# kendallsullivan/mcmc_spec

Hardware: AMD Instinct MI355X
Metric: walker log-likelihood evals/sec (whole node) (higher is better)
Workload: dtype f64

## Files before the change

mcmc_spec_amd/csrc/msx.hip:

```cpp

#include <dlfcn.h>
#include <hip/hip_runtime.h>
#include <math.h>
#include <stdint.h>
#include <stdio.h>
#include <string.h>

#include <algorithm>
#include <array>
#include <mutex>
#include <type_traits>
#include <string>
#include <vector>

#include "../../include/msx.h"

#include "dev_types.h"
#include "wave_ops.h"
#include "blend.h"
#include "recipe.h"
#include "median.h"
#include "logprob_kernel.h"
#include "move_kernels.h"
#include "tempered_kernels.h"
// ... 34 lines not shown
    bool pf_ok = false;
    bool pf256_ok = false;
    bool model_in_global = false;
    void *rccl_comm = nullptr;
    hipStream_t comm_stream = nullptr;
    hipEvent_t ev_ready = nullptr;
    hipEvent_t ev_done[4] = {nullptr, nullptr, nullptr, nullptr};
    int comm_world = 0, comm_rank = 0;
    std::vector<msx_ctx *> loop_peers;
    hipEvent_t loop_eval_done = nullptr;
    hipEvent_t loop_copied = nullptr;
    double *d_model_scratch = nullptr;
    SegPart *d_segparts = nullptr;
    unsigned long long *d_seg_flag = nullptr;
    int nseg = 1;
    int64_t scratch_rows = 0;
    int32_t path = 0;
    int32_t broaden_placement = 0;
    double *d_raw_win = nullptr;
    int64_t raw_i0 = 0, raw_n = 0;
    int raw_lx = 0;
    double raw_dx = 0.0, raw_sigma = 0.0;
    bool grid_rotated = false;
    int32_t ncomp = 1;
    InpathRec *d_inp_rec = nullptr;
    double *d_inp_tmp = nullptr, *d_inp_given = nullptr;
    const int64_t *d_pix_lo = nullptr;
    int64_t inp_rows = 0, inp_gstride = 0;
    int64_t pair_rows = 0;
    int64_t pair_min_walkers = 4096;
    int32_t *d_pair_plan = nullptr;
    PairItem *d_pair_items = nullptr;
    PairRec *d_pair_singles = nullptr;
    int32_t *h_pair_stats = nullptr;
    int64_t pair_auto_launches = 0;
    int32_t linked = -1;
    bool linked_poisoned = false;
    bool recipe_fast = false;
    unsigned char *d_recipe_block = nullptr;
    struct SamplerRun *smp = nullptr;
    struct OptRun *opt_run = nullptr;
    struct TemperedRun *tmp = nullptr;
    bool smp_overlap_launch = false;
    bool probe_launch = false;
    int32_t last_form = 0;
    int32_t smp_overlap_policy = -1;
    int32_t store_dtype = MSX_STORE_F64;
    bool store_f32 = false;
    uint64_t prob_gen = 0;
    std::vector<struct msx_group *> groups;
    bool products_staged = false;
    ProdMember PM;
    ProdMember *d_prod_member = nullptr;
    std::vector<void *> prod_allocs;
    char *d_prod_buf = nullptr;
    size_t prod_buf_bytes = 0;
};
static void sampler_free(msx_ctx *c);
static void opt_run_free(msx_ctx *c);
static void tempered_free(msx_ctx *c);

struct msx_group {
    int device = 0;
    std::string err;
    std::vector<msx_ctx *> members;
    std::vector<uint64_t> gen;
// ... 94 lines not shown
    if (count <= 0) {
        HIP_TRY(c, hipMalloc((void **)out, 16));
        if (track) track->push_back(*out);
        return MSX_OK;
    }
    HIP_TRY(c, hipMalloc((void **)out, sizeof(T) * count));
    if (track) track->push_back(*out);
    HIP_TRY(c, hipMemcpy(*out, host, sizeof(T) * count, hipMemcpyHostToDevice));
    return MSX_OK;
}

void free_problem(msx_ctx *c) {
    sampler_free(c);
    opt_run_free(c);
    tempered_free(c);
    for (msx_group *g : c->groups) group_run_drain(g);
    ++c->prob_gen;
    for (void *p : c->prob_allocs) (void)hipFree(p);
    c->prob_allocs.clear();
    c->problem_staged = false;
    for (void *p : c->prod_allocs) (void)hipFree(p);
    c->prod_allocs.clear();
    if (c->d_prod_buf) (void)hipFree(c->d_prod_buf);
    c->d_prod_buf = nullptr; c->prod_buf_bytes = 0;
    c->d_prod_member = nullptr;
    c->products_staged = false;
    if (c->d_opt_flux) (void)hipFree(c->d_opt_flux);
    if (c->d_opt_med) (void)hipFree(c->d_opt_med);
    c->d_opt_flux = c->d_opt_med = nullptr;
    c->opt_chains = 0;
    if (c->h_pair_stats) (void)hipHostFree(c->h_pair_stats);
    c->h_pair_stats = nullptr;
    void *sp[] = {c->d_model_scratch, c->d_segparts, c->d_seg_flag, c->d_pair_plan, c->d_pair_items, c->d_pair_singles,
                  c->d_inp_rec, c->d_inp_tmp, c->d_inp_given};
    for (void *p : sp)
        if (p) (void)hipFree(p);
    c->d_segparts = nullptr; c->d_seg_flag = nullptr; c->d_model_scratch = nullptr; c->scratch_rows = 0;
    c->d_pair_plan = nullptr; c->d_pair_items = nullptr; c->d_pair_singles = nullptr; c->pair_rows = 0;
    c->linked_poisoned = false;
    c->d_inp_rec = nullptr; c->d_inp_tmp = c->d_inp_given = nullptr; c->d_pix_lo = nullptr; c->inp_rows = 0;
}

void free_grid(msx_ctx *c) {
    void *ptrs[] = {c->d_grid, c->d_wl, c->d_kgrid, c->d_teff, c->d_logg, c->d_present};
    for (void *p : ptrs)
        if (p) (void)hipFree(p);
    c->d_grid = c->d_wl = c->d_kgrid = c->d_teff = c->d_logg = nullptr;
    c->d_present = nullptr;
    if (c->d_raw_win) (void)hipFree(c->d_raw_win);
    c->d_raw_win = nullptr; c->raw_n = 0;
    c->grid_rotated = false;
    c->ncomp = 1;
    c->grid_staged = false;
}

int64_t grid_rows(const msx_ctx *c) { return (int64_t)c->ncomp * c->nt * c->ng; }

int conv_taps(double mean_wl, double dx, double resolution, double maxsig, double *sigma_out, int *lx_out) {
    const double fwhm = 1.0 / resolution * mean_wl;
    const double sigma = fwhm / (2.0 * sqrt(2.0 * log(2.0)));
    const int lx = (int)(((sigma * maxsig) / dx) * 2.0) + 1;
    *sigma_out = sigma;
    *lx_out = lx;
    return lx;
}

int check_even_spacing(msx_ctx *c, const double *wl, int64_t n) {
    double mx = -INFINITY, mn = INFINITY, sum = 0.0;
    for (int64_t i = 1; i < n; ++i) {
        const double d = wl[i] - wl[i - 1];
        mx = d > mx ? d : mx;
// ... 152 lines not shown
    return {(const void *)logprob_kernel<NS, T, GM, SH, PF, LK, R32, FULL, GIVEN>, NS, T, GM, SH, PF, LK, R32, FULL, GIVEN, what};
}
const Variant kVariants[] = {
    variant<2, 256, false, false, false, false>("three workgroups per CU"),
    variant<2, 256, false, true, false, false>("two per CU, four pixels per lane and trip"),
    variant<2, 256, false, true, true, false>("two per CU, u / flux staged in LDS during the recipe, four pixels per lane and trip"),
    variant<2, 512, false, false, false, false>("one workgroup per CU, four pixels per lane and trip"),
    variant<2, 512, false, true, false, false>("<= 128 VGPRs: two workgroups fit a CU; rows one star at a time"),
    variant<2, 512, false, false, true, false>("one workgroup per CU, u / flux staged in LDS during the recipe, four pixels per lane and trip"),
    variant<3, 256, false, false, false, false>("three workgroups per CU"),
    variant<3, 512, false, false, false, false>("one workgroup per CU, four pixels per lane and trip"),
    variant<3, 512, false, false, true, false>("one workgroup per CU, u / flux staged in LDS during the recipe, four pixels per lane and trip"),
    variant<2, 512, false, false, false, true>("one workgroup per walker and 8192-pixel segment; partial sums and histogram counters exchanged inside the launch; the segment's data flux staged in LDS; four pixels per lane and trip"),
    variant<3, 512, false, false, false, true>("one workgroup per walker and 8192-pixel segment; partial sums and histogram counters exchanged inside the launch; the segment's data flux staged in LDS; four pixels per lane and trip"),
    variant<2, 512, true, false, false, false>("model vector in global memory (spectra beyond the LDS), sub-batched"),
    variant<3, 512, true, false, false, false>("model vector in global memory (spectra beyond the LDS), sub-batched"),
    variant<2, 256, false, false, false, false, true>("three workgroups per CU; R table stored in float32"),
    variant<2, 256, false, true, false, false, true>("two per CU, four pixels per lane and trip; R table stored in float32"),
    variant<2, 256, false, true, true, false, true>("two per CU, u / flux staged in LDS during the recipe, four pixels per lane and trip; R table stored in float32"),
    variant<2, 512, false, false, false, false, true>("one workgroup per CU, four pixels per lane and trip; R table stored in float32"),
    variant<2, 512, false, true, false, false, true>("<= 128 VGPRs: two workgroups fit a CU; rows one star at a time; R table stored in float32"),
    variant<2, 512, false, false, true, false, true>("one workgroup per CU, u / flux staged in LDS during the recipe, four pixels per lane and trip; R table stored in float32"),
    variant<2, 256, false, false, false, false, false, 3>("three workgroups per CU; whole trips, no clamps"),
    variant<2, 256, false, true, false, false, false, 3>("two per CU, four pixels per lane and trip; whole trips, no clamps"),
    variant<2, 256, false, true, true, false, false, 3>("two per CU, u / flux staged in LDS during the recipe, four pixels per lane and trip; whole trips, no clamps"),
    variant<2, 512, false, false, true, false, false, 2>("one workgroup per CU, u / flux staged in LDS during the recipe, four pixels per lane and trip; whole trips, no clamps in the chi^2 pass"),
    variant<2, 512, false, true, false, false, false, 2>("<= 128 VGPRs: two workgroups fit a CU; rows one star at a time; whole trips, no clamps in the chi^2 pass"),
    variant<2, 512, false, false, true, false, true, 2>("float32-stored grid table R; one workgroup per CU, u / flux staged in LDS; whole trips, no clamps in the chi^2 pass"),
    variant<2, 512, false, false, false, true, false, 2>("linked: one workgroup per walker and 8192-pixel segment; whole trips, no clamps in the chi^2 pass"),
    variant<2, 512, false, false, false, false, false, 0, true>("model values given by the in-path broadening kernels; four pixels per lane and trip"),
};

struct PairVariant {
    void (*fn)(const double *, const unsigned char *, int, int, int64_t, double, double, const int32_t *, DevProblem, double *, int32_t *);
    int nt;
    bool full;
};
const PairVariant kPairVariants[] = {
    {logprob_pair_kernel<512, 2, true>, 2, false},
    {logprob_pair_kernel<512, 2, true, true>, 2, true},
    {logprob_pair_kernel<512, 4, true>, 4, false},
    {logprob_pair_kernel<512, 4, true, true>, 4, true},
};

const Variant *find_variant(const Variant &want, bool whole) {
    const Variant *hit = nullptr;
    for (const Variant &v : kVariants)
        if (v.ns == want.ns && v.threads == want.threads && v.gm == want.gm && v.sh == want.sh && v.pf == want.pf &&
            v.lk == want.lk && v.r32 == want.r32 && v.given == want.given && (v.full == 0 || whole) && (!hit || v.full != 0))
            hit = &v;
    return hit;
}

struct LaunchPlan {
    int64_t rows = 0;
    int64_t m = 0;
    int block = 0;
    const Variant *v = nullptr;
    const PairVariant *pv = nullptr;
    const void *fn = nullptr;
    int threads = 0;
    size_t dyn_lds = 0;
    int64_t grid = 0;
    int64_t bytes = 0;
};


// ... 201 lines not shown
            pf = pf && g->pf_ok[m];
            pf256 = pf256 && g->pf256_ok[m];
        }
    const int B = block_threads > 0 ? block_threads : pick_block(g->cus, total, npix);
    bool whole = true;
    for (int m = 0; m < k; ++m)
        if (counts[m] > 0) whole = whole && whole_trips(g->probs[m], 2 * (int64_t)B);
    FusedShape want = fused_shape(g->cus, total, npix, B, shared512, pf, pf256);
    const int ns = g->nspec == 2 ? 2 : 3;
    const GroupVariant *hit = nullptr;
    for (int attempt = 0; attempt < 2 && !hit; ++attempt) {
        if (attempt == 1) want.sh = want.pf = false;
        for (const GroupVariant &v : kGroupVariants)
            if (v.ns == ns && v.threads == B && v.sh == want.sh && v.pf == want.pf && (v.full == 0 || whole) && (!hit || v.full != 0))
                hit = &v;
    }
    return hit ? group_plan_lds(g, counts, total, hit) : GroupPlan();
}

GroupPlan group_plan_lds(const msx_group *g, const int64_t *counts, int64_t total, const GroupVariant *v) {
    GroupPlan pl;
    pl.v = v;
    double bytes = 0.0;
    for (int m = 0; m < (int)g->members.size(); ++m) {
        if (counts[m] <= 0) continue;
        pl.dyn_lds = std::max(pl.dyn_lds, fused_dyn_lds(g->probs[m], v->pf));
        bytes += (double)fused_bytes(g->probs[m], v->pf, false) * (double)counts[m];
    }
    pl.bytes = (int64_t)(bytes / (double)total + 0.5);
    return pl;
}

int launch_pair(msx_ctx *c, const DevProblem &P, const LaunchArgs &A, const LaunchPlan &pl) {
    const int32_t *plan = c->d_pair_plan;
    hipLaunchKernelGGL(pair_plan_kernel, dim3((unsigned)((A.n + kPlanThreads - 1) / kPlanThreads)), dim3(kPlanThreads), 0, A.s, A.theta,
                       (const unsigned char *)c->d_recipe_block, A.niso_nt, A.ng_mode_fast, (int64_t)A.n, P.tmin, P.tmax,
                       c->d_pair_plan, c->d_pair_items, c->d_pair_singles, A.logp, A.status, c->h_pair_stats, P);
    HIP_TRY(c, hipGetLastError());
    hipLaunchKernelGGL(pl.pv->fn, dim3((unsigned)pl.grid), dim3((unsigned)pl.threads), 0, A.s, A.theta, (const unsigned char *)c->d_recipe_block,
                       A.niso_nt, A.ng_mode_fast, (int64_t)A.n, P.tmin, P.tmax, plan, P, A.logp, A.status);
    HIP_TRY(c, hipGetLastError());
    return MSX_OK;
}

hipError_t raise_one(const void *kernel) {
    hipFuncAttributes at;
    hipError_t e = hipFuncGetAttributes(&at, kernel);
    if (e != hipSuccess) return e;
    const int room = (160 * 1024 - (int)at.sharedSizeBytes) & ~15;
    return hipFuncSetAttribute(kernel, hipFuncAttributeMaxDynamicSharedMemorySize, room);
}
hipError_t raise_all() {
    hipError_t e = hipSuccess;
    for (const Variant &v : kVariants)
        if (e == hipSuccess && !v.gm) e = raise_one(v.fn);
    for (const GroupVariant &v : kGroupVariants) {
        if (e == hipSuccess) e = raise_one(v.fn);
        if (e == hipSuccess && v.smp_fn) e = raise_one(v.smp_fn);
    }
    if (e == hipSuccess) e = raise_one((const void *)broaden_conv_kernel);
    if (e == hipSuccess) e = raise_one((const void *)rot_broaden_kernel<true>);
    return e;
}
constexpr int kMaxDevices = 64;
int raise_dynamic_lds_limits(msx_ctx *c) {
    static std::mutex mu;
    static bool done[kMaxDevices] = {};
    if (c->device < 0 || c->device >= kMaxDevices)
        return fail(c, MSX_ERR_INVALID, "device index beyond the per-device table of dynamic-LDS limits (64 devices)");
    std::lock_guard<std::mutex> lock(mu);
    if (done[c->device]) return MSX_OK;
    HIP_TRY(c, raise_all());
    done[c->device] = true;
// ... 584 lines not shown
    c->nseg = (int)((npair + kSegElems - 1) / kSegElems);
    const bool can_link = c->nseg >= 2 && c->nseg <= 8;
    P.linked_fault = 0;
    if (model_in_global || can_link) {
        int64_t budget = 96ll << 20;
        if (const char *e = getenv("MSX_SCRATCH_MB")) budget = std::max<int64_t>(1, atoll(e)) << 20;
        int64_t sb = budget / (int64_t)(sizeof(double) * p->npix);
        sb = std::max<int64_t>(256, std::min<int64_t>(sb, 16384));
        HIP_TRY(c, hipMalloc((void **)&c->d_model_scratch, sizeof(double) * sb * p->npix));
        c->scratch_rows = sb;
        P.model_scratch = c->d_model_scratch;
        if (can_link) {
            HIP_TRY(c, hipMalloc((void **)&c->d_segparts, sizeof(SegPart) * sb * c->nseg));
            P.segparts = c->d_segparts;
            HIP_TRY(c, hipMalloc((void **)&c->d_seg_flag, sizeof(unsigned long long) * (sb + 1)));
            HIP_TRY(c, hipMemset(c->d_seg_flag, 0, sizeof(unsigned long long) * (sb + 1)));
            P.seg_flag = c->d_seg_flag;
            P.linked_poison = reinterpret_cast<int32_t *>(c->d_seg_flag + sb);
        }
    }
    c->linked_poisoned = false;
    if (p->nspec == 2 && p->npix <= kPairMaxPix && c->recipe_fast && !p->no_spectrum) {
        const int64_t rows = 16384;
        HIP_TRY(c, hipMalloc((void **)&c->d_model_scratch, sizeof(double) * kPairSpillRows * p->npix));
        P.model_scratch = c->d_model_scratch;
        const size_t plan_bytes = sizeof(int32_t) * (size_t)(kPairHdrInts + kPairSpillRows);
        HIP_TRY(c, hipMalloc((void **)&c->d_pair_plan, plan_bytes));
        HIP_TRY(c, hipMemset(c->d_pair_plan, 0, plan_bytes));
        P.pair_lease = c->d_pair_plan + kPairHdrInts;
        HIP_TRY(c, hipMalloc((void **)&c->d_pair_items, sizeof(PairItem) * (size_t)((rows + 1) / 2)));
        HIP_TRY(c, hipMalloc((void **)&c->d_pair_singles, sizeof(PairRec) * (size_t)rows));
        P.pair_items = c->d_pair_items;
        P.pair_singles = c->d_pair_singles;
        HIP_TRY(c, hipHostMalloc((void **)&c->h_pair_stats, 2 * sizeof(int32_t), hipHostMallocDefault));
        c->h_pair_stats[0] = 1; c->h_pair_stats[1] = 0;
        c->pair_auto_launches = 0;
        c->pair_rows = rows;
        {
            const int64_t cus = c->prop.multiProcessorCount > 0 ? c->prop.multiProcessorCount : 256;
            c->pair_min_walkers = (p->npix > 3072 ? 8 : 12) * cus;
        }
        if (const char *e = getenv("MSX_PAIR_MIN")) c->pair_min_walkers = atoll(e) > 0 ? std::max<int64_t>(2, atoll(e)) : INT64_MAX;
    }
#ifdef MSX_STAMPS
    {
        unsigned long long *st = nullptr;
        HIP_TRY(c, hipMalloc((void **)&st, sizeof(unsigned long long) * 16 * 65536)); tr.push_back(st);
        HIP_TRY(c, hipMemset(st, 0, sizeof(unsigned long long) * 16 * 65536));
        P.stamps = st;
    }
#endif
    {
        unsigned long long *cp = nullptr;
        HIP_TRY(c, hipMalloc((void **)&cp, sizeof(unsigned long long) * 4 * kProbeWalkers)); tr.push_back(cp);
        HIP_TRY(c, hipMemset(cp, 0, sizeof(unsigned long long) * 4 * kProbeWalkers));
        P.clk_probe = cp;
    }
    c->problem_staged = true;
    return MSX_OK;
}

#ifdef MSX_STAMPS
int msx_diag_read_med_stamps(msx_ctx *c, int64_t n, unsigned long long *out) {
    if (!c || n > 65536) return MSX_ERR_INVALID;
    HIP_TRY(c, hipDeviceSynchronize());
    HIP_TRY(c, hipMemcpyFromSymbol(out, HIP_SYMBOL(g_med_stamps), sizeof(unsigned long long) * 8 * n));
    return MSX_OK;
}
int msx_diag_read_stamps(msx_ctx *c, int64_t n, unsigned long long *out) {
    if (!c || !c->problem_staged || n > 65536) return MSX_ERR_INVALID;
    HIP_TRY(c, hipDeviceSynchronize());
    HIP_TRY(c, hipMemcpy(out, c->P.stamps, sizeof(unsigned long long) * 16 * n, hipMemcpyDeviceToHost));
    return MSX_OK;
// ... 3176 lines not shown
```

mcmc_spec_amd/csrc/pair_kernel.h:

```cpp
#ifndef MSX_PAIR_KERNEL_H
#define MSX_PAIR_KERNEL_H

namespace {

constexpr int kPairMaxPix = 4096;
constexpr int kPairSpillRows = 1024;
constexpr int kPairHdrInts = 8;

template <int I, int N, class F>
__device__ __forceinline__ void static_for(F &&f) {
    if constexpr (I < N) {
        f(std::integral_constant<int, I>{});
        static_for<I + 1, N>(f);
    }
}

template <int MAXT, int NT, bool RED, bool FULL = false>
__global__ void __launch_bounds__(MAXT, MAXT == 256 ? 2 : 4)
logprob_pair_kernel(const double *theta, const unsigned char *__restrict__ rblk, int niso_nt, int ng_mode_fast, int64_t n,
                    double gate_tmin, double gate_tmax, const int32_t *__restrict__ plan, DevProblem P,
                    double *__restrict__ logp, int32_t *__restrict__ status) {
    constexpr int NS = 2, ndim = 6, NC = 8, B = MAXT, nw = B >> 6;
    (void)rblk; (void)niso_nt; (void)n; (void)gate_tmin; (void)gate_tmax;
    static_assert(NT * MAXT * 2 <= kPairMaxPix, "model values per lane");
    constexpr int vk = kMaxWaves / nw;
    constexpr int G = MAXT == 256 ? NC : 4;
    static_assert(MAXT == 256 || MAXT == 512, "256 or 512 threads");
    __shared__ WalkerDesc D[2];
    __shared__ BlockScratch S[2];
    __shared__ double red[2][3][nw][kWave];
    __shared__ double e2tab[kExp2Tab];
    struct WalkerLoc { double pc[3]; LogbinSel Q; int appl; unsigned int fsel, fspan; };
    __shared__ WalkerLoc Loc[2];
    const int mode = (ng_mode_fast >> 8) & 0xff;
    const int tid0 = threadIdx.x, lane0 = tid0 & 63, wave0 = tid0 >> 6;
    const PairRec *rec[2];
    bool is_pair;
    {
        const int2 cnt = *reinterpret_cast<const int2 *>(plan);
        const int b = (int)blockIdx.x, sb = b - cnt.x;
        if (sb >= cnt.y) return;
        is_pair = sb < 0;
        rec[0] = is_pair ? &P.pair_items[b].r[0] : P.pair_singles + sb;
        rec[1] = is_pair ? &P.pair_items[b].r[1] : rec[0];
    }
    const int npix = (int)P.npix;
    const int ne = (int)P.npair;

    if (wave0 < 2 && lane0 < NC) {
        const PairRec *R = rec[wave0];
        D[wave0].node[lane0] = R->node[lane0];
        D[wave0].w[lane0] = R->w[lane0];
        if (lane0 == 0) { D[wave0].redc = R->redc; D[wave0].lp = R->lp; D[wave0].chi_extra = R->chi_extra; D[wave0].ncorner = R->walker; }
    }
    fill_exp2_table(e2tab, tid0 - (B - kWave));
    for (int i = tid0; i < kLogBins; i += B) { S[0].hist[i] = 0; S[1].hist[i] = 0; }
    if (tid0 < 2) { S[tid0].cand_n = 0; S[tid0].has_second = 0; }
    __syncthreads();
    const int64_t wkv[2] = {D[0].ncorner, is_pair ? D[1].ncorner : -1};
    const bool act0 = true, act1 = is_pair;
    bool same = act1;
    if (same) {
#pragma unroll
        for (int c = 0; c < NC; ++c) same = same && D[0].node[c] == D[1].node[c];
    }
    const bool need_two = (npix & 1) == 0;

    auto body = [&](auto two_c, const int sa, const int sb, const bool again) __attribute__((always_inline)) {
        constexpr bool two = decltype(two_c)::value;
        constexpr int NSLOT = two ? 2 : 1;
        const int tid = tid0, lane = lane0, wave = wave0;
        const int64_t wk0 = wkv[sa], wk1 = wkv[sb];
        const WalkerDesc &Da = D[sa], &Db = D[sb];
        if (again) {
            for (int i = tid; i < kLogBins; i += B) S[0].hist[i] = 0;
            if (tid == 0) { S[0].cand_n = 0; S[0].has_second = 0; }
            __syncthreads();
        }

        const double2 *rows_r[NC];
        const float2 *rows_h[NC];
        double wA[NC], wB[NC];
        float wfA[NC], wfB[NC];
#pragma unroll
        for (int c = 0; c < NC; ++c) {
            const int64_t off = (int64_t)__builtin_amdgcn_readfirstlane(Da.node[c]) * ne;
            rows_r[c] = P.r2 + off;
            rows_h[c] = P.h2 + off;
            wA[c] = uniform_f64(Da.w[c]);
            wfA[c] = uniform_f32((float)wA[c]);
            wB[c] = uniform_f64(Db.w[c]);
            wfB[c] = uniform_f32((float)wB[c]);
        }
        const double redcA = uniform_f64(Da.redc), redcB = uniform_f64(Db.redc);
        const bool reddenA = redcA != 0.0, reddenB = two && redcB != 0.0;
        double2 m[2][NT];
        double qa[2][vk][3];
        unsigned int fmin[2] = {~0u, ~0u}, fmax[2] = {0u, 0u};
        auto finish_elem = [&](auto s_c, auto j_c, const double2 m2, const double2 f2, const double2 u2, const int ec,
                               const bool live) __attribute__((always_inline)) {
            constexpr int s = decltype(s_c)::value, j = decltype(j_c)::value;
            constexpr int kbase = MAXT == 256 ? 2 * (j & 1) : 0;
            const int pa = ((ec >> 8) << 9) | (ec & 255), pb = pa + 256;
            const bool ok[2] = {FULL || (live && pa < npix), FULL || (live && pb < npix)};
            const double mm[2] = {m2.x, m2.y}, ff[2] = {f2.x, f2.y}, uu[2] = {u2.x, u2.y};
// ... 108 lines not shown
            for (int i = 0; i < 3; ++i) q[i] = S[s].q[0][i];
            unsigned int f0 = (unsigned int)S[s].kmin[0], f1 = (unsigned int)S[s].kmax[0];
            for (int x = 1; x < nw; ++x) {
                f0 = (unsigned int)S[s].kmin[x] < f0 ? (unsigned int)S[s].kmin[x] : f0;
                f1 = (unsigned int)S[s].kmax[x] > f1 ? (unsigned int)S[s].kmax[x] : f1;
            }
            fit_coefs(P, q, c0, c1, c2);
            LogbinSel Qs = {0u, 0u, 0u, 0u};
            bool ap = frange_applicable(f0, f1);
            if (ap) ap = logbin_locate_h<MAXT>(npix, f0, S[s], &Qs);
            if (lane == 0) {
                Loc[s].pc[0] = c0; Loc[s].pc[1] = c1; Loc[s].pc[2] = c2;
                Loc[s].Q = Qs;
                Loc[s].appl = ap;
                const unsigned int fsel = f0 + ((Qs.sel_p - f0) & (unsigned int)(kLogBins - 1));
                const unsigned int fnxt = f0 + ((Qs.nxt_p - f0) & (unsigned int)(kLogBins - 1));
                Loc[s].fsel = ap ? fsel : 1u;
                Loc[s].fspan = ap ? fnxt - fsel : 0u;
            }
        });
        __syncthreads();
        double pc[2][3];
        bool bad[2] = {false, false}, appl[2];
        LogbinSel Q[2];
        unsigned int fsel[2], fspan[2];
        static_for<0, NSLOT>([&](auto s_c) __attribute__((always_inline)) {
            constexpr int s = decltype(s_c)::value;
            pc[s][0] = Loc[s].pc[0]; pc[s][1] = Loc[s].pc[1]; pc[s][2] = Loc[s].pc[2];
            Q[s] = Loc[s].Q;
            appl[s] = Loc[s].appl != 0;
            fsel[s] = Loc[s].fsel; fspan[s] = Loc[s].fspan;
        });

        double acc[2][vk];
#pragma unroll
        for (int s = 0; s < NSLOT; ++s)
#pragma unroll
            for (int k = 0; k < vk; ++k) acc[s][k] = 0.0;
        auto pass_trip = [&](auto j_c) __attribute__((always_inline)) {
            constexpr int j = decltype(j_c)::value;
            constexpr int kbase = MAXT == 256 ? 2 * (j & 1) : 0;
            int tj = tid;
            asm volatile("" : "+v"(tj));
            const int e = j * B + tj;
            const int ec = (FULL || e < ne) ? e : ne - 1;
            const unsigned int o16 = (unsigned int)ec << 4;
            const double2 nv = ld_off(P.iv2, o16), cu = ld_off(P.u2, o16), cf = ld_off(P.f2, o16);
            const int pa = ((e >> 8) << 9) | (e & 255);
            const bool livep[2] = {FULL || (e < ne && pa < npix), FULL || (e < ne && pa + 256 < npix)};
            const double uu[2] = {cu.x, cu.y}, ff[2] = {cf.x, cf.y}, ee[2] = {nv.x, nv.y};
            static_for<0, NSLOT>([&](auto s_c) __attribute__((always_inline)) {
                constexpr int s = decltype(s_c)::value;
                const double xv[2] = {m[s][j].x, m[s][j].y};
#pragma unroll
                for (int u = 0; u < 2; ++u) {
                    acc[s][kbase + u] += chi_term(pc[s][0], pc[s][1], pc[s][2], uu[u], ff[u], ee[u], xv[u], livep[u]);
                    const unsigned int fx = (unsigned int)__double2hiint(xv[u]) >> 12;
                    if (appl[s] && livep[u] && fx - fsel[s] <= fspan[s])
                        S[s].cand[atomicAdd(&S[s].cand_n, 1u)] = key_of(xv[u]);
                }
            });
            __builtin_amdgcn_sched_barrier(0);
        };
        static_for<0, NT>(pass_trip);
        red[0][0][wave][lane] = lane_partial<vk>(acc[0]);
        if (two) red[1][0][wave][lane] = lane_partial<vk>(acc[1]);
// ... 45 lines not shown
                for (;;) {
                    if (atomicCAS(P.pair_lease + lease, 0, 1) == 0) { got = true; break; }
                    if (wall_clock64() - t0 > kHandoverTicks) break;
                    __builtin_amdgcn_s_sleep(8);
                }
                S[s].meet_state = got ? 1u : 0u;
            }
            __syncthreads();
            if (S[s].meet_state == 0u) { lost[s] = true; return; }
            double *row = P.model_scratch + (int64_t)lease * npix;
            auto spill = [&](auto j_c) __attribute__((always_inline)) {
                constexpr int j = decltype(j_c)::value;
                const int e = j * B + tid;
                const int pa = ((e >> 8) << 9) | (e & 255);
                if (e < ne && pa < npix) row[pa] = m[s][j].x;
                if (e < ne && pa + 256 < npix) row[pa + 256] = m[s][j].y;
            };
            static_for<0, NT>(spill);
            for (int i = tid; i < kBins; i += B) S[s].hist[i] = 0;
            __threadfence_block();
            __syncthreads();
            NoElem no_elem;
            bool unused = false;
            med[s] = block_median<MAXT>(row, npix, kmin, kmax, S[s], NoSide(), no_elem, &unused);
            __syncthreads();
            if (tid == 0) atomicExch(P.pair_lease + lease, 0);
        });

        static_for<0, NSLOT>([&](auto s_c) __attribute__((always_inline)) {
            constexpr int s = decltype(s_c)::value;
            if (wave != s) return;
            const double tot = reduce_published<MAXT>(&red[s][0][0][0], lane);
            if (lane == 0) {
                const WalkerDesc &Dw = s == 0 ? D[sa] : D[sb];
                const int64_t wk = s == 0 ? wk0 : wk1;
                double out;
                if (bad[s]) {
                    out = mode == MSX_MODE_CHISQ ? NAN : -INFINITY;
                } else {
                    const double total = fused_total(P, tot, P.median_flux, med[s], npix, Dw.chi_extra);
                    out = value_of_total(mode, total, Dw.lp);
                }
                logp[wk] = lost[s] ? nan_with_status(MSX_W_HANDOVER) : out;
                status[wk] = lost[s] ? MSX_W_HANDOVER : MSX_W_OK;
            }
        });
    };
    if (same) {
        body(std::true_type{}, 0, 1, false);
    } else {
        if (act0) body(std::false_type{}, 0, 0, false);
        __syncthreads();
        if (act1) body(std::false_type{}, 1, 1, true);
    }
}

constexpr int kPlanThreads = 256;
constexpr int kPlanCells = 12;
constexpr int kPlanSortMax = 2048;

__device__ __forceinline__ void stage_scalar_tables(const unsigned char *__restrict__ rblk, const DevProblem &P, int niso, int nt, int ng,
                                                    ScalarTabs &T, ScalarPriorTabs &TP) {
    __shared__ double s_isot[kPlanIsoPad], s_isol[kPlanIsoPad], s_teff[kPlanNodePad + 1], s_logg[kPlanNodePad + 1];
    __shared__ double4 s_isopack[kPlanIsoPad];
    __shared__ double s_ave[kPlanIsoPad], s_avm[2 * kWave], s_avs[2 * kWave];
    __shared__ unsigned int s_pmask[kWave];
    static_assert(kPlanThreads == kPlanIsoPad, "one table entry per thread");
    const int tid = threadIdx.x;
    const double *g_isot = reinterpret_cast<const double *>(rblk + kRbIsoT);
    const double4 *g_pack = reinterpret_cast<const double4 *>(rblk + kRbIsoPack);
    const double *g_teff = reinterpret_cast<const double *>(rblk + kRbTeff), *g_logg = reinterpret_cast<const double *>(rblk + kRbLogg);
    const int nav = P.nav;
    const int ii = tid < niso ? tid : niso - 1, it = tid < nt ? tid : nt - 1, ig = tid < ng ? tid : ng - 1;
    const int ie = tid < nav + 1 ? tid : 0, ia = tid < nav ? tid : 0;
// ... 8 lines not shown
    s_ave[tid] = (nav > 0 && tid < nav + 1) ? v_ave : INFINITY;
    if (tid < 2 * kWave) { s_avm[tid] = v_avm; s_avs[tid] = v_avs; }
    if (tid <= kPlanNodePad) { s_teff[tid] = tid < nt ? v_teff : INFINITY; s_logg[tid] = tid < ng ? v_logg : INFINITY; }
    if (tid < kWave) s_pmask[tid] = tid < nt ? v_mask : 0u;
    T = ScalarTabs{s_isot, s_teff, s_logg, s_isopack, s_pmask, s_ave, niso, nt, ng, nav, P.node_stride};
    TP = ScalarPriorTabs{s_isot, s_isol, s_avm, s_avs};
}

__device__ __forceinline__ void plan_wave_pairs(unsigned long long tag, int lane, int *partner_lane, bool *leftover) {
    *partner_lane = -1;
    *leftover = false;
    unsigned long long rem = __ballot(tag != 0ull);
    unsigned long long mygrp = 0ull;
    for (int trip = 0; rem != 0ull && trip < kPlanCells; ++trip) {
        const int leader = __ffsll((long long)rem) - 1;
        const unsigned long long ltag = readlane_u64(tag, leader);
        const unsigned long long grp = __ballot(tag == ltag);
        mygrp = (tag == ltag) ? grp : mygrp;
        rem &= ~grp;
    }
    if (mygrp != 0ull) {
        const int r = __popcll(mygrp & ((1ull << lane) - 1ull));
        if ((r & 1) == 0) {
            const unsigned long long nxt = lane < 63 ? (mygrp & ~((2ull << lane) - 1ull)) : 0ull;
            if (nxt != 0ull) *partner_lane = __ffsll((long long)nxt) - 1; else *leftover = true;
        }
    }
    if ((rem >> lane) & 1ull) *leftover = true;
}

__global__ void __launch_bounds__(kPlanThreads)
pair_plan_kernel(const double *__restrict__ theta, const unsigned char *__restrict__ rblk, int niso_nt, int ng_mode_fast, int64_t n,
                 double gate_tmin, double gate_tmax, int32_t *__restrict__ plan, PairItem *__restrict__ pair_items,
                 PairRec *__restrict__ single_items, double *__restrict__ logp, int32_t *__restrict__ status, int32_t *__restrict__ host_stats, DevProblem P) {
    constexpr int NS = 2, ndim = 6;
    __shared__ unsigned long long s_cards[kPlanSortMax];
    __shared__ int2 s_pairs[kPlanSortMax / 2];
    __shared__ unsigned long long s_left[kPlanSortMax];
    __shared__ int s_nc, s_np, s_nl, s_ns, s_basep, s_basel;
    static_assert(kPlanThreads == kPlanIsoPad, "one table entry per thread");
    const int niso = niso_nt & 0xffff, nt = niso_nt >> 16;
    const int ng = ng_mode_fast & 0xff, mode = (ng_mode_fast >> 8) & 0xff;
    const GateArgs gates = {gate_tmin, gate_tmax, ((ng_mode_fast >> 18) & 1) != 0, ((ng_mode_fast >> 19) & 1) != 0};
    const int tid = threadIdx.x, lane = tid & 63;
    __shared__ int s_where[kPlanThreads];
    s_where[tid] = -1;
#ifdef MSX_STAMPS
    if (tid == 0) msx_stamp_off = 0;
#endif
    MSX_STAMP(P, blockIdx.x, 0);
    const int64_t i = (int64_t)blockIdx.x * kPlanThreads + tid;
    const bool mine = i < n;
    double t[ndim];
#pragma unroll
    for (int k = 0; k < ndim; ++k) t[k] = mine ? theta[i * ndim + k] : 0.0;
    ScalarTabs T;
    ScalarPriorTabs TP;
    stage_scalar_tables(rblk, P, niso, nt, ng, T, TP);
    if (tid == 0) { s_nc = 0; s_np = 0; s_nl = 0; s_ns = 0; }
    __syncthreads();
    MSX_STAMP(P, blockIdx.x, 1);
    unsigned long long tag = 0ull;
    PairRec mrec;
    int node[NS * 4], iso_lo[NS] = {0, 0}, av_bin = 0;
    double w[NS * 4];
    BandRows band_pre;
    if (mine) {
        double redc;
        const int st = recipe_scalar2(gates, T, mode, t, node, w, &redc, iso_lo, &av_bin);
        MSX_STAMP(P, blockIdx.x, 2);
        if (st != MSX_W_OK) {
            logp[i] = (st > MSX_W_REJECT) ? nan_with_status(st) : -INFINITY;
            status[i] = st;
        } else {
            PairRec *R = &mrec;
#pragma unroll
            for (int c = 0; c < NS * 4; ++c) { R->w[c] = w[c]; R->node[c] = node[c]; }
            R->redc = redc;
            R->walker = (int32_t)i;
            R->pad = 0;
            band_rows_first(P, node, band_pre);
            unsigned long long h = 0x9E3779B97F4A7C15ull;
#pragma unroll
            for (int c = 0; c < NS * 4; ++c) {
                h ^= (unsigned long long)(unsigned int)node[c] + 0x9E3779B97F4A7C15ull + (h << 6) + (h >> 2);
                h *= 0xBF58476D1CE4E5B9ull;
                h ^= h >> 31;
            }
            tag = (h >> 24) | 1ull;
        }
    }
    int partner_lane;
    bool leftover;
    plan_wave_pairs(tag, lane, &partner_lane, &leftover);
    const int partner_walker = __shfl((int)i, partner_lane >= 0 ? partner_lane : lane);
    const unsigned long long below = (1ull << lane) - 1ull;

    {
        const unsigned long long bp = __ballot(partner_lane >= 0), bl = __ballot(leftover), bs = 0ull;
        int basep = 0, basel = 0, bases = 0;
        if (lane == 0) {
            if (bp) basep = atomicAdd(&s_np, __popcll(bp));
            if (bl) basel = atomicAdd(&s_nc, __popcll(bl));
            if (bs) bases = atomicAdd(&s_ns, __popcll(bs));
        }
        basep = __builtin_amdgcn_readfirstlane(basep);
        basel = __builtin_amdgcn_readfirstlane(basel);
        bases = __builtin_amdgcn_readfirstlane(bases);
        if (partner_lane >= 0) s_pairs[basep + __popcll(bp & below)] = make_int2((int)i, partner_walker);
        if (leftover) s_cards[basel + __popcll(bl & below)] = (tag << 24) | (unsigned long long)(i + 1);
        (void)bases;
    }
    __syncthreads();
    MSX_STAMP(P, blockIdx.x, 3);
    int nc = s_nc;
    const int nsingle = s_ns;
    unsigned long long *src = s_cards, *dst = s_cards + kPlanSortMax / 2;
    for (int round = 0; round < 3 && nc > 1; ++round) {
        const bool one_wave = nc <= kWave;
        if (tid == 0) s_nl = 0;
        __syncthreads();
        const int k = tid;
        const unsigned long long cd = k < nc ? src[k] : 0ull;
        int pl;
        bool lo;
        plan_wave_pairs(cd >> 24, lane, &pl, &lo);
        const unsigned long long other = __shfl(cd, pl >= 0 ? pl : lane);
        const unsigned long long bp = __ballot(pl >= 0), bl = __ballot(lo);
        int basep = 0, basel = 0;
        if (lane == 0) {
            if (bp) basep = atomicAdd(&s_np, __popcll(bp));
            if (bl) basel = atomicAdd(&s_nl, __popcll(bl));
        }
        basep = __builtin_amdgcn_readfirstlane(basep);
        basel = __builtin_amdgcn_readfirstlane(basel);
        if (pl >= 0) s_pairs[basep + __popcll(bp & below)] = make_int2((int)(cd & 0xffffffull) - 1, (int)(other & 0xffffffull) - 1);
        if (lo) dst[basel + __popcll(bl & below)] = cd;
        __syncthreads();
        const int left = s_nl;
        if (left == nc) break;
        nc = left;
        unsigned long long *t_ = src; src = dst; dst = t_;
        if (one_wave) break;
    }
    __syncthreads();
    for (int k = tid; k < nc; k += kPlanThreads) s_left[nsingle + k] = src[k];
    if (tid == 0) s_nl = nc;
    __syncthreads();
    MSX_STAMP(P, blockIdx.x, 4);
    const int np = s_np, nl = s_nl;
    int gbase = 0;
    int tid_v = tid;
    asm volatile("" : "+v"(tid_v));
    if (tid < 2) gbase = atomicAdd(&plan[2 + tid_v], tid == 0 ? np : nsingle + nl);
    MSX_STAMP(P, blockIdx.x, 5);
    if (tag != 0ull) {
        mrec.lp = prior_terms_scalar2(P, TP, mode, t, av_bin, iso_lo);
        MSX_STAMP(P, blockIdx.x, 6);
        mrec.chi_extra = band_terms_scalar2(P, mode, t, node, w, band_pre);
        MSX_STAMP(P, blockIdx.x, 7);
    }
    if (tid == 0) s_basep = gbase;
    if (tid == 1) s_basel = gbase;
    int ticket = -1;
    if (tid < 1) ticket = atomicAdd(&plan[4 + tid_v], 1);
    __syncthreads();
    const int base = blockIdx.x * kPlanThreads;
    for (int k = tid; k < np; k += kPlanThreads) {
        s_where[s_pairs[k].x - base] = (s_basep + k) << 1;
        s_where[s_pairs[k].y - base] = ((s_basep + k) << 1) | 1;
    }
    for (int k = tid; k < nsingle + nl; k += kPlanThreads) s_where[(int)(s_left[k] & 0xffffffull) - 1 - base] = -2 - (s_basel + k);
    __syncthreads();
    if (tag != 0ull) {
        const int wh = s_where[tid];
        PairRec *dst = wh >= 0 ? &pair_items[wh >> 1].r[wh & 1] : single_items + (-2 - wh);
        *dst = mrec;
    }
    MSX_STAMP(P, blockIdx.x, 8);
    if (tid == 0 && ticket == (int)gridDim.x - 1) {
        const int np_all = atomicExch(&plan[2], 0), ns_all = atomicExch(&plan[3], 0);
        plan[0] = np_all;
        plan[1] = ns_all;
        if (host_stats) {
            __hip_atomic_store(host_stats, np_all, __ATOMIC_RELAXED, __HIP_MEMORY_SCOPE_SYSTEM);
            __hip_atomic_store(host_stats + 1, ns_all, __ATOMIC_RELAXED, __HIP_MEMORY_SCOPE_SYSTEM);
        }
        atomicExch(&plan[4], 0);
    }
    MSX_STAMP(P, blockIdx.x, 9);
}

}

#endif
```

Before: 17.76 million.

## Split pair-plan kernel into pairing and prior/band-term blocks, drop last-block ticket

```diff
diff --git a/mcmc_spec_amd/csrc/msx.hip b/mcmc_spec_amd/csrc/msx.hip
--- a/mcmc_spec_amd/csrc/msx.hip
+++ b/mcmc_spec_amd/csrc/msx.hip
@@ -90,6 +90,7 @@
     int32_t *d_pair_plan = nullptr;
     PairItem *d_pair_items = nullptr;
     PairRec *d_pair_singles = nullptr;
+    double2 *d_pair_side = nullptr;
     int32_t *h_pair_stats = nullptr;
     int64_t pair_auto_launches = 0;
     int32_t linked = -1;
@@ -250,11 +251,11 @@
     if (c->h_pair_stats) (void)hipHostFree(c->h_pair_stats);
     c->h_pair_stats = nullptr;
     void *sp[] = {c->d_model_scratch, c->d_segparts, c->d_seg_flag, c->d_pair_plan, c->d_pair_items, c->d_pair_singles,
-                  c->d_inp_rec, c->d_inp_tmp, c->d_inp_given};
+                  c->d_pair_side, c->d_inp_rec, c->d_inp_tmp, c->d_inp_given};
     for (void *p : sp)
         if (p) (void)hipFree(p);
     c->d_segparts = nullptr; c->d_seg_flag = nullptr; c->d_model_scratch = nullptr; c->scratch_rows = 0;
-    c->d_pair_plan = nullptr; c->d_pair_items = nullptr; c->d_pair_singles = nullptr; c->pair_rows = 0;
+    c->d_pair_plan = nullptr; c->d_pair_items = nullptr; c->d_pair_singles = nullptr; c->d_pair_side = nullptr; c->pair_rows = 0;
     c->linked_poisoned = false;
     c->d_inp_rec = nullptr; c->d_inp_tmp = c->d_inp_given = nullptr; c->d_pix_lo = nullptr; c->inp_rows = 0;
 }
@@ -473,7 +474,7 @@
 };
 
 struct PairVariant {
-    void (*fn)(const double *, const unsigned char *, int, int, int64_t, double, double, const int32_t *, DevProblem, double *, int32_t *);
+    void (*fn)(const double *, const unsigned char *, int, int, int64_t, double, double, int32_t *, DevProblem, double *, int32_t *, const double2 *, int32_t *);
     int nt;
     bool full;
 };
@@ -741,13 +742,13 @@
 }
 
 int launch_pair(msx_ctx *c, const DevProblem &P, const LaunchArgs &A, const LaunchPlan &pl) {
-    const int32_t *plan = c->d_pair_plan;
-    hipLaunchKernelGGL(pair_plan_kernel, dim3((unsigned)((A.n + kPlanThreads - 1) / kPlanThreads)), dim3(kPlanThreads), 0, A.s, A.theta,
+    const unsigned plan_blocks = (unsigned)((A.n + kPlanThreads - 1) / kPlanThreads);
+    hipLaunchKernelGGL(pair_plan_kernel, dim3(2 * plan_blocks), dim3(kPlanThreads), 0, A.s, A.theta,
                        (const unsigned char *)c->d_recipe_block, A.niso_nt, A.ng_mode_fast, (int64_t)A.n, P.tmin, P.tmax,
-                       c->d_pair_plan, c->d_pair_items, c->d_pair_singles, A.logp, A.status, c->h_pair_stats, P);
+                       c->d_pair_plan, c->d_pair_items, c->d_pair_singles, A.logp, A.status, c->d_pair_side, P);
     HIP_TRY(c, hipGetLastError());
     hipLaunchKernelGGL(pl.pv->fn, dim3((unsigned)pl.grid), dim3((unsigned)pl.threads), 0, A.s, A.theta, (const unsigned char *)c->d_recipe_block,
-                       A.niso_nt, A.ng_mode_fast, (int64_t)A.n, P.tmin, P.tmax, plan, P, A.logp, A.status);
+                       A.niso_nt, A.ng_mode_fast, (int64_t)A.n, P.tmin, P.tmax, c->d_pair_plan, P, A.logp, A.status, c->d_pair_side, c->h_pair_stats);
     HIP_TRY(c, hipGetLastError());
     return MSX_OK;
 }
@@ -1398,13 +1399,15 @@
         HIP_TRY(c, hipMalloc((void **)&c->d_pair_singles, sizeof(PairRec) * (size_t)rows));
         P.pair_items = c->d_pair_items;
         P.pair_singles = c->d_pair_singles;
+        HIP_TRY(c, hipMalloc((void **)&c->d_pair_side, sizeof(double2) * (size_t)rows));
+        HIP_TRY(c, hipMemset(c->d_pair_side, 0, sizeof(double2) * (size_t)rows));
         HIP_TRY(c, hipHostMalloc((void **)&c->h_pair_stats, 2 * sizeof(int32_t), hipHostMallocDefault));
         c->h_pair_stats[0] = 1; c->h_pair_stats[1] = 0;
         c->pair_auto_launches = 0;
         c->pair_rows = rows;
         {
             const int64_t cus = c->prop.multiProcessorCount > 0 ? c->prop.multiProcessorCount : 256;
-            c->pair_min_walkers = (p->npix > 3072 ? 8 : 12) * cus;
+            c->pair_min_walkers = (p->npix > 3072 ? 6 : 8) * cus;
         }
         if (const char *e = getenv("MSX_PAIR_MIN")) c->pair_min_walkers = atoll(e) > 0 ? std::max<int64_t>(2, atoll(e)) : INT64_MAX;
     }
diff --git a/mcmc_spec_amd/csrc/pair_kernel.h b/mcmc_spec_amd/csrc/pair_kernel.h
--- a/mcmc_spec_amd/csrc/pair_kernel.h
+++ b/mcmc_spec_amd/csrc/pair_kernel.h
@@ -18,8 +18,9 @@
 template <int MAXT, int NT, bool RED, bool FULL = false>
 __global__ void __launch_bounds__(MAXT, MAXT == 256 ? 2 : 4)
 logprob_pair_kernel(const double *theta, const unsigned char *__restrict__ rblk, int niso_nt, int ng_mode_fast, int64_t n,
-                    double gate_tmin, double gate_tmax, const int32_t *__restrict__ plan, DevProblem P,
-                    double *__restrict__ logp, int32_t *__restrict__ status) {
+                    double gate_tmin, double gate_tmax, int32_t *plan, DevProblem P,
+                    double *__restrict__ logp, int32_t *__restrict__ status, const double2 *__restrict__ side,
+                    int32_t *__restrict__ host_stats) {
     constexpr int NS = 2, ndim = 6, NC = 8, B = MAXT, nw = B >> 6;
     (void)rblk; (void)niso_nt; (void)n; (void)gate_tmin; (void)gate_tmax;
     static_assert(NT * MAXT * 2 <= kPairMaxPix, "model values per lane");
@@ -37,9 +38,21 @@
     const PairRec *rec[2];
     bool is_pair;
     {
-        const int2 cnt = *reinterpret_cast<const int2 *>(plan);
-        const int b = (int)blockIdx.x, sb = b - cnt.x;
-        if (sb >= cnt.y) return;
+        int epoch = 0;
+        if (blockIdx.x == 0) epoch = plan[2];
+        const int4 c4 = *reinterpret_cast<const int4 *>(plan + 4);
+        const int np_all = c4.x + c4.z, ns_all = c4.y + c4.w;
+        if (blockIdx.x == 0 && tid0 == 0) {
+            plan[0] = np_all;
+            plan[1] = ns_all;
+            plan[2] = epoch + 1;
+            if (host_stats) {
+                __hip_atomic_store(host_stats, np_all, __ATOMIC_RELAXED, __HIP_MEMORY_SCOPE_SYSTEM);
+                __hip_atomic_store(host_stats + 1, ns_all, __ATOMIC_RELAXED, __HIP_MEMORY_SCOPE_SYSTEM);
+            }
+        }
+        const int b = (int)blockIdx.x, sb = b - np_all;
+        if (sb >= ns_all) return;
         is_pair = sb < 0;
         rec[0] = is_pair ? &P.pair_items[b].r[0] : P.pair_singles + sb;
         rec[1] = is_pair ? &P.pair_items[b].r[1] : rec[0];
@@ -51,13 +64,12 @@
         const PairRec *R = rec[wave0];
         D[wave0].node[lane0] = R->node[lane0];
         D[wave0].w[lane0] = R->w[lane0];
-        if (lane0 == 0) { D[wave0].redc = R->redc; D[wave0].lp = R->lp; D[wave0].chi_extra = R->chi_extra; D[wave0].ncorner = R->walker; }
+        if (lane0 == 0) { D[wave0].redc = R->redc; D[wave0].ncorner = R->walker; }
     }
     fill_exp2_table(e2tab, tid0 - (B - kWave));
     for (int i = tid0; i < kLogBins; i += B) { S[0].hist[i] = 0; S[1].hist[i] = 0; }
     if (tid0 < 2) { S[tid0].cand_n = 0; S[tid0].has_second = 0; }
     __syncthreads();
-    const int64_t wkv[2] = {D[0].ncorner, is_pair ? D[1].ncorner : -1};
     const bool act0 = true, act1 = is_pair;
     bool same = act1;
     if (same) {
@@ -70,7 +82,6 @@
         constexpr bool two = decltype(two_c)::value;
         constexpr int NSLOT = two ? 2 : 1;
         const int tid = tid0, lane = lane0, wave = wave0;
-        const int64_t wk0 = wkv[sa], wk1 = wkv[sb];
         const WalkerDesc &Da = D[sa], &Db = D[sb];
         if (again) {
             for (int i = tid; i < kLogBins; i += B) S[0].hist[i] = 0;
@@ -245,6 +256,7 @@
             fsel[s] = Loc[s].fsel; fspan[s] = Loc[s].fspan;
         });
 
+        const double2 sd = side[D[(two && wave == 1) ? sb : sa].ncorner];
         double acc[2][vk];
 #pragma unroll
         for (int s = 0; s < NSLOT; ++s)
@@ -356,14 +368,13 @@
             if (wave != s) return;
             const double tot = reduce_published<MAXT>(&red[s][0][0][0], lane);
             if (lane == 0) {
-                const WalkerDesc &Dw = s == 0 ? D[sa] : D[sb];
-                const int64_t wk = s == 0 ? wk0 : wk1;
+                const int64_t wk = D[s == 0 ? sa : sb].ncorner;
                 double out;
                 if (bad[s]) {
                     out = mode == MSX_MODE_CHISQ ? NAN : -INFINITY;
                 } else {
-                    const double total = fused_total(P, tot, P.median_flux, med[s], npix, Dw.chi_extra);
-                    out = value_of_total(mode, total, Dw.lp);
+                    const double total = fused_total(P, tot, P.median_flux, med[s], npix, sd.y);
+                    out = value_of_total(mode, total, sd.x);
                 }
                 logp[wk] = lost[s] ? nan_with_status(MSX_W_HANDOVER) : out;
                 status[wk] = lost[s] ? MSX_W_HANDOVER : MSX_W_OK;
@@ -438,12 +449,17 @@
 __global__ void __launch_bounds__(kPlanThreads)
 pair_plan_kernel(const double *__restrict__ theta, const unsigned char *__restrict__ rblk, int niso_nt, int ng_mode_fast, int64_t n,
                  double gate_tmin, double gate_tmax, int32_t *__restrict__ plan, PairItem *__restrict__ pair_items,
-                 PairRec *__restrict__ single_items, double *__restrict__ logp, int32_t *__restrict__ status, int32_t *__restrict__ host_stats, DevProblem P) {
+                 PairRec *__restrict__ single_items, double *__restrict__ logp, int32_t *__restrict__ status, double2 *__restrict__ side, DevProblem P) {
     constexpr int NS = 2, ndim = 6;
+    const int nblk = (int)(gridDim.x >> 1);
+    const bool term_block = (int)blockIdx.x >= nblk;
+    const int blk = term_block ? (int)blockIdx.x - nblk : (int)blockIdx.x;
+    const int epoch = plan[2];
     __shared__ unsigned long long s_cards[kPlanSortMax];
     __shared__ int2 s_pairs[kPlanSortMax / 2];
     __shared__ unsigned long long s_left[kPlanSortMax];
-    __shared__ int s_nc, s_np, s_nl, s_ns, s_basep, s_basel;
+    __shared__ int s_np, s_nl, s_basep, s_basel;
+    __shared__ int s_wc[2][kPlanThreads / kWave];
     static_assert(kPlanThreads == kPlanIsoPad, "one table entry per thread");
     const int niso = niso_nt & 0xffff, nt = niso_nt >> 16;
     const int ng = ng_mode_fast & 0xff, mode = (ng_mode_fast >> 8) & 0xff;
@@ -455,7 +471,7 @@
     if (tid == 0) msx_stamp_off = 0;
 #endif
     MSX_STAMP(P, blockIdx.x, 0);
-    const int64_t i = (int64_t)blockIdx.x * kPlanThreads + tid;
+    const int64_t i = (int64_t)blk * kPlanThreads + tid;
     const bool mine = i < n;
     double t[ndim];
 #pragma unroll
@@ -463,18 +479,31 @@
     ScalarTabs T;
     ScalarPriorTabs TP;
     stage_scalar_tables(rblk, P, niso, nt, ng, T, TP);
-    if (tid == 0) { s_nc = 0; s_np = 0; s_nl = 0; s_ns = 0; }
+    if (tid == 0) { s_np = 0; s_nl = 0; }
     __syncthreads();
     MSX_STAMP(P, blockIdx.x, 1);
     unsigned long long tag = 0ull;
     PairRec mrec;
     int node[NS * 4], iso_lo[NS] = {0, 0}, av_bin = 0;
     double w[NS * 4];
-    BandRows band_pre;
+    double redc = 0.0;
+    int st = MSX_W_REJECT;
+    if (mine) st = recipe_scalar2(gates, T, mode, t, node, w, &redc, iso_lo, &av_bin);
+    MSX_STAMP(P, blockIdx.x, 2);
+    if (term_block) {
+        if (st == MSX_W_OK) {
+            BandRows band_pre;
+            band_rows_first(P, node, band_pre);
+            const double lp = prior_terms_scalar2(P, TP, mode, t, av_bin, iso_lo);
+            MSX_STAMP(P, blockIdx.x, 3);
+            const double chi_extra = band_terms_scalar2(P, mode, t, node, w, band_pre);
+            MSX_STAMP(P, blockIdx.x, 4);
+            side[i] = make_double2(lp, chi_extra);
+        }
+        MSX_STAMP(P, blockIdx.x, 5);
+        return;
+    }
     if (mine) {
-        double redc;
-        const int st = recipe_scalar2(gates, T, mode, t, node, w, &redc, iso_lo, &av_bin);
-        MSX_STAMP(P, blockIdx.x, 2);
         if (st != MSX_W_OK) {
             logp[i] = (st > MSX_W_REJECT) ? nan_with_status(st) : -INFINITY;
             status[i] = st;
@@ -485,7 +514,7 @@
             R->redc = redc;
             R->walker = (int32_t)i;
             R->pad = 0;
-            band_rows_first(P, node, band_pre);
+            R->lp = R->chi_extra = 0.0;
             unsigned long long h = 0x9E3779B97F4A7C15ull;
 #pragma unroll
             for (int c = 0; c < NS * 4; ++c) {
@@ -502,55 +531,57 @@
     const int partner_walker = __shfl((int)i, partner_lane >= 0 ? partner_lane : lane);
     const unsigned long long below = (1ull << lane) - 1ull;
 
+    auto plan_card = [&](const unsigned long long *buf, const int *cnt, int k, int *total) __attribute__((always_inline)) {
+        const int p1 = cnt[0], p2 = p1 + cnt[1], p3 = p2 + cnt[2];
+        const int v = (k >= p1) + (k >= p2) + (k >= p3);
+        const int first = v == 0 ? 0 : (v == 1 ? p1 : (v == 2 ? p2 : p3));
+        *total = p3 + cnt[3];
+        return k < *total ? buf[v * kWave + (k - first)] : 0ull;
+    };
+    static_assert(kPlanThreads == 4 * kWave, "plan_card: four waves");
+    const int wave = tid >> 6;
     {
-        const unsigned long long bp = __ballot(partner_lane >= 0), bl = __ballot(leftover), bs = 0ull;
-        int basep = 0, basel = 0, bases = 0;
+        const unsigned long long bp = __ballot(partner_lane >= 0), bl = __ballot(leftover);
+        int basep = 0;
         if (lane == 0) {
             if (bp) basep = atomicAdd(&s_np, __popcll(bp));
-            if (bl) basel = atomicAdd(&s_nc, __popcll(bl));
-            if (bs) bases = atomicAdd(&s_ns, __popcll(bs));
+            s_wc[0][wave] = __popcll(bl);
         }
         basep = __builtin_amdgcn_readfirstlane(basep);
-        basel = __builtin_amdgcn_readfirstlane(basel);
-        bases = __builtin_amdgcn_readfirstlane(bases);
         if (partner_lane >= 0) s_pairs[basep + __popcll(bp & below)] = make_int2((int)i, partner_walker);
-        if (leftover) s_cards[basel + __popcll(bl & below)] = (tag << 24) | (unsigned long long)(i + 1);
-        (void)bases;
+        if (leftover) s_cards[wave * kWave + __popcll(bl & below)] = (tag << 24) | (unsigned long long)(i + 1);
     }
     __syncthreads();
     MSX_STAMP(P, blockIdx.x, 3);
-    int nc = s_nc;
-    const int nsingle = s_ns;
-    unsigned long long *src = s_cards, *dst = s_cards + kPlanSortMax / 2;
+    const int nsingle = 0;
+    int cur = 0, nc;
+    unsigned long long cd = plan_card(s_cards, s_wc[0], tid, &nc);
     for (int round = 0; round < 3 && nc > 1; ++round) {
         const bool one_wave = nc <= kWave;
-        if (tid == 0) s_nl = 0;
-        __syncthreads();
-        const int k = tid;
-        const unsigned long long cd = k < nc ? src[k] : 0ull;
+        unsigned long long *dst = s_cards + (cur ^ 1) * (kPlanSortMax / 2);
         int pl;
         bool lo;
         plan_wave_pairs(cd >> 24, lane, &pl, &lo);
         const unsigned long long other = __shfl(cd, pl >= 0 ? pl : lane);
         const unsigned long long bp = __ballot(pl >= 0), bl = __ballot(lo);
-        int basep = 0, basel = 0;
+        int basep = 0;
         if (lane == 0) {
             if (bp) basep = atomicAdd(&s_np, __popcll(bp));
-            if (bl) basel = atomicAdd(&s_nl, __popcll(bl));
+            s_wc[cur ^ 1][wave] = __popcll(bl);
         }
         basep = __builtin_amdgcn_readfirstlane(basep);
-        basel = __builtin_amdgcn_readfirstlane(basel);
         if (pl >= 0) s_pairs[basep + __popcll(bp & below)] = make_int2((int)(cd & 0xffffffull) - 1, (int)(other & 0xffffffull) - 1);
-        if (lo) dst[basel + __popcll(bl & below)] = cd;
+        if (lo) dst[wave * kWave + __popcll(bl & below)] = cd;
         __syncthreads();
-        const int left = s_nl;
+        int left;
+        const unsigned long long nxt = plan_card(dst, s_wc[cur ^ 1], tid, &left);
         if (left == nc) break;
         nc = left;
-        unsigned long long *t_ = src; src = dst; dst = t_;
+        cd = nxt;
+        cur ^= 1;
         if (one_wave) break;
     }
-    __syncthreads();
-    for (int k = tid; k < nc; k += kPlanThreads) s_left[nsingle + k] = src[k];
+    if (tid < nc) s_left[nsingle + tid] = cd;
     if (tid == 0) s_nl = nc;
     __syncthreads();
     MSX_STAMP(P, blockIdx.x, 4);
@@ -558,43 +589,25 @@
     int gbase = 0;
     int tid_v = tid;
     asm volatile("" : "+v"(tid_v));
-    if (tid < 2) gbase = atomicAdd(&plan[2 + tid_v], tid == 0 ? np : nsingle + nl);
+    const int set = 4 + 2 * (epoch & 1);
+    if (tid < 2) gbase = atomicAdd(&plan[set + tid_v], tid == 0 ? np : nsingle + nl);
+    if (blk == 0 && tid < 2) plan[(set ^ 2) + tid_v] = 0;
     MSX_STAMP(P, blockIdx.x, 5);
-    if (tag != 0ull) {
-        mrec.lp = prior_terms_scalar2(P, TP, mode, t, av_bin, iso_lo);
-        MSX_STAMP(P, blockIdx.x, 6);
-        mrec.chi_extra = band_terms_scalar2(P, mode, t, node, w, band_pre);
-        MSX_STAMP(P, blockIdx.x, 7);
-    }
+    const int base = blk * kPlanThreads;
+    for (int k = tid; k < np; k += kPlanThreads) {
+        s_where[s_pairs[k].x - base] = k << 1;
+        s_where[s_pairs[k].y - base] = (k << 1) | 1;
+    }
+    for (int k = tid; k < nsingle + nl; k += kPlanThreads) s_where[(int)(s_left[k] & 0xffffffull) - 1 - base] = -2 - k;
     if (tid == 0) s_basep = gbase;
     if (tid == 1) s_basel = gbase;
-    int ticket = -1;
-    if (tid < 1) ticket = atomicAdd(&plan[4 + tid_v], 1);
-    __syncthreads();
-    const int base = blockIdx.x * kPlanThreads;
-    for (int k = tid; k < np; k += kPlanThreads) {
-        s_where[s_pairs[k].x - base] = (s_basep + k) << 1;
-        s_where[s_pairs[k].y - base] = ((s_basep + k) << 1) | 1;
-    }
-    for (int k = tid; k < nsingle + nl; k += kPlanThreads) s_where[(int)(s_left[k] & 0xffffffull) - 1 - base] = -2 - (s_basel + k);
     __syncthreads();
     if (tag != 0ull) {
         const int wh = s_where[tid];
-        PairRec *dst = wh >= 0 ? &pair_items[wh >> 1].r[wh & 1] : single_items + (-2 - wh);
+        PairRec *dst = wh >= 0 ? &pair_items[s_basep + (wh >> 1)].r[wh & 1] : single_items + (s_basel + (-2 - wh));
         *dst = mrec;
     }
-    MSX_STAMP(P, blockIdx.x, 8);
-    if (tid == 0 && ticket == (int)gridDim.x - 1) {
-        const int np_all = atomicExch(&plan[2], 0), ns_all = atomicExch(&plan[3], 0);
-        plan[0] = np_all;
-        plan[1] = ns_all;
-        if (host_stats) {
-            __hip_atomic_store(host_stats, np_all, __ATOMIC_RELAXED, __HIP_MEMORY_SCOPE_SYSTEM);
-            __hip_atomic_store(host_stats + 1, ns_all, __ATOMIC_RELAXED, __HIP_MEMORY_SCOPE_SYSTEM);
-        }
-        atomicExch(&plan[4], 0);
-    }
-    MSX_STAMP(P, blockIdx.x, 9);
+    MSX_STAMP(P, blockIdx.x, 6);
 }
 
 }
```

After: 17.78 million, median of 3. No clear change (+0.1%).
